# rakhimovv/lvt

Measured on AMD Instinct MI355X. Metric: video-clips/sec/node (VQVAE+DSFVT train step, BAIR 64x64x16), higher is better.
Workload: dtype f32

## Files before the change

### lvt_amd/csrc/gemm_engine.hip

```cpp
#include "lvt_common.h"
#include "epilogue_fast.h"
#include <string.h>
#include <stdlib.h>
#include <stdint.h>
#include <type_traits>

typedef float f32x16 __attribute__((ext_vector_type(16)));

#define BK 32
#define NTHREADS 256

enum { A_KPLAIN = 0, A_MPLAIN = 1, A_CONV_K = 2, A_CONVT_K = 3, A_CONV_M = 4, A_ONEHOT_M = 5, A_PATCH = 6, A_PATCHT = 7 };
enum { B_KPLAIN = 0, B_NPLAIN = 1, B_CONVT_W = 2 };

struct KParams {
    int M, N, K;
    const float *A; long long lda; int a_kb; long long a_skb;
    const float *B; long long ldb; int b_kb; long long b_skb;
    float *C; long long ldc; long long c_plane;
    int batch_inner;
    long long sA_o, sA_i, sB_o, sB_i, sC_o, sC_i;
    float alpha; int flags;
    const float *bias; const float *res; long long ldr; const float *mask; long long ldm;
    int splits; int k_per_split; float *partial; long long partial_stride;
    int vec_epi;
    float *colsum_partial;
    const float *a_amax, *b_amax;
    const float *a_amax2, *b_amax2;
    float *c_amax;
    lvt_conv_geom g;
    const char *b_img;
    int Tq, Hq, Wq;
    int jT, jH, jW;
    const long long *oh_idx; long long oh_bstride, oh_pstride; int oh_P, oh_V; int oh_off[32];
};

__device__ __forceinline__ float4 ldg4(const float *p) { return *reinterpret_cast<const float4 *>(p); }

__device__ __forceinline__ unsigned cvt_pk_bf16(float lo, float hi) {
    unsigned r;
    asm("v_cvt_pk_bf16_f32 %0, %1, %2" : "=v"(r) : "v"(lo), "v"(hi));
    return r;
}
__device__ __forceinline__ float bf_lo(unsigned p) { return __uint_as_float(p << 16); }
__device__ __forceinline__ float bf_hi(unsigned p) { return __uint_as_float(p & 0xffff0000u); }
__device__ __forceinline__ void split3(const float4 v, uint2 &p1, uint2 &p2, uint2 &p3) {
    p1.x = cvt_pk_bf16(v.x, v.y); p1.y = cvt_pk_bf16(v.z, v.w);
    const float r0 = v.x - bf_lo(p1.x), r1 = v.y - bf_hi(p1.x), r2 = v.z - bf_lo(p1.y), r3 = v.w - bf_hi(p1.y);
    p2.x = cvt_pk_bf16(r0, r1); p2.y = cvt_pk_bf16(r2, r3);
    const float s0 = r0 - bf_lo(p2.x), s1 = r1 - bf_hi(p2.x), s2 = r2 - bf_lo(p2.y), s3 = r3 - bf_hi(p2.y);
    p3.x = cvt_pk_bf16(s0, s1); p3.y = cvt_pk_bf16(s2, s3);
}
#define HLD 40
template <int ROWS> __device__ __forceinline__ int hrow(int m) {
    if (ROWS >= 128) {
        const int r = (m & ~127) + ((m & 3) << 5) + ((m & 127) >> 2);
        return r * HLD + (r >> 5) * 32;
    }
    return m * HLD;
}
template <int ROWS> struct HPlane { static constexpr int SIZE = ROWS * HLD + (ROWS >= 128 ? ROWS : 0); };
template <int ROWS> __device__ __forceinline__ void store_split_k(unsigned short *lds, int row, int k4, const float4 v) {
    uint2 p1, p2, p3;
    split3(v, p1, p2, p3);
    unsigned short *d = lds + hrow<ROWS>(row) + k4;
    *reinterpret_cast<uint2 *>(d) = p1;
    *reinterpret_cast<uint2 *>(d + HPlane<ROWS>::SIZE) = p2;
    *reinterpret_cast<uint2 *>(d + 2 * HPlane<ROWS>::SIZE) = p3;
}
template <int ROWS> __device__ __forceinline__ void store_split_m(unsigned short *lds, int row4, int k, const float4 v) {
    uint2 p[3];
    split3(v, p[0], p[1], p[2]);
#pragma unroll
    for (int q = 0; q < 3; ++q) {
        unsigned short *d = lds + q * HPlane<ROWS>::SIZE + k;
        d[hrow<ROWS>(row4)] = (unsigned short)(p[q].x & 0xffffu); d[hrow<ROWS>(row4 + 1)] = (unsigned short)(p[q].x >> 16);
        d[hrow<ROWS>(row4 + 2)] = (unsigned short)(p[q].y & 0xffffu); d[hrow<ROWS>(row4 + 3)] = (unsigned short)(p[q].y >> 16);
    }
}
template <int ROWS> __device__ __forceinline__ void store_split_block(unsigned short *lds, int row4, int k4, const float4 *v) {
    store_split_k<ROWS>(lds, row4 + 0, k4, make_float4(v[0].x, v[1].x, v[2].x, v[3].x));
    store_split_k<ROWS>(lds, row4 + 1, k4, make_float4(v[0].y, v[1].y, v[2].y, v[3].y));
    store_split_k<ROWS>(lds, row4 + 2, k4, make_float4(v[0].z, v[1].z, v[2].z, v[3].z));
    store_split_k<ROWS>(lds, row4 + 3, k4, make_float4(v[0].w, v[1].w, v[2].w, v[3].w));
}
__device__ __forceinline__ float4 zero4() { return make_float4(0.f, 0.f, 0.f, 0.f); }

typedef float f32x2 __attribute__((ext_vector_type(2)));
typedef _Float16 f16x2v __attribute__((ext_vector_type(2)));
__device__ __forceinline__ float f16_mix_lo(unsigned h, float k, float c) {
    float r;
    asm("v_fma_mix_f32 %0, %1, %2, %3 op_sel:[0,0,0] op_sel_hi:[1,0,0]" : "=v"(r) : "v"(h), "v"(k), "v"(c));
    return r;
}
__device__ __forceinline__ float f16_mix_hi(unsigned h, float k, float c) {
    float r;
    asm("v_fma_mix_f32 %0, %1, %2, %3 op_sel:[1,0,0] op_sel_hi:[1,0,0]" : "=v"(r) : "v"(h), "v"(k), "v"(c));
    return r;
}
template <int LOSCALE>
__device__ __forceinline__ void f16_split_pair(float a, float b, float s, unsigned &ph, unsigned &pl) {
    const f32x2 v = {a, b};
    ph = __builtin_bit_cast(unsigned, __builtin_convertvector(v * s, f16x2v));
    const f32x2 t2 = v * (s * (float)LOSCALE);
    const f32x2 r = {f16_mix_lo(ph, -(float)LOSCALE, t2.x), f16_mix_hi(ph, -(float)LOSCALE, t2.y)};
    pl = __builtin_bit_cast(unsigned, __builtin_convertvector(r, f16x2v));
}
__device__ __forceinline__ void split2(const float4 v, const float s, uint2 &ph, uint2 &pl) {
    f16_split_pair<2048>(v.x, v.y, s, ph.x, pl.x);
    f16_split_pair<2048>(v.z, v.w, s, ph.y, pl.y);
}
__device__ __forceinline__ unsigned f16_pair_mix(float a, float b, float s) {
    unsigned r;
    asm("v_fma_mixlo_f16 %0, %1, %2, 0\n\tv_fma_mixhi_f16 %0, %3, %2, 0" : "=&v"(r) : "v"(a), "v"(s), "v"(b));
    return r;
}
__device__ __forceinline__ void split2_lean(const float4 v, const float s, uint2 &ph, uint2 &pl) {
    ph.x = f16_pair_mix(v.x, v.y, s); ph.y = f16_pair_mix(v.z, v.w, s);
    pl.x = f16_pair_mix(f16_mix_lo(ph.x, -1.f, v.x * s), f16_mix_hi(ph.x, -1.f, v.y * s), 2048.f);
    pl.y = f16_pair_mix(f16_mix_lo(ph.y, -1.f, v.z * s), f16_mix_hi(ph.y, -1.f, v.w * s), 2048.f);
}
__device__ __forceinline__ float lvt_f16_scale(const float *amax, int &unscale, const float *amax2 = nullptr) {
    if (!amax) return 1.f;
    unsigned bits = __float_as_uint(*amax);
    if (amax2) bits = max(bits, __float_as_uint(*amax2));
    const int eb = (int)((bits >> 23) & 0xffu);
    int se = 268 - eb;
    se = se < 2 ? 2 : (se > 252 ? 252 : se);
    unscale -= se - 127;
    return __uint_as_float((unsigned)se << 23);
}
template <int ROWS, int LEAN = 0> __device__ __forceinline__ void store_split2_k(unsigned short *lds, int row, int k4, const float4 v, float s) {
    uint2 ph, pl;
    if (LEAN) split2_lean(v, s, ph, pl);
    else split2(v, s, ph, pl);
    unsigned short *d = lds + hrow<ROWS>(row) + k4;
    *reinterpret_cast<uint2 *>(d) = ph;
    *reinterpret_cast<uint2 *>(d + HPlane<ROWS>::SIZE) = pl;
}
template <int ROWS, int LEAN = 0> __device__ __forceinline__ void store_split2_m(unsigned short *lds, int row4, int k, const float4 v, float s) {
    uint2 p[2];
    if (LEAN) split2_lean(v, s, p[0], p[1]);
    else split2(v, s, p[0], p[1]);
#pragma unroll
    for (int q = 0; q < 2; ++q) {
        unsigned short *d = lds + q * HPlane<ROWS>::SIZE + k;
        d[hrow<ROWS>(row4)] = (unsigned short)(p[q].x & 0xffffu); d[hrow<ROWS>(row4 + 1)] = (unsigned short)(p[q].x >> 16);
        d[hrow<ROWS>(row4 + 2)] = (unsigned short)(p[q].y & 0xffffu); d[hrow<ROWS>(row4 + 3)] = (unsigned short)(p[q].y >> 16);
    }
}
template <int ROWS, int LEAN = 0> __device__ __forceinline__ void store_split2_block(unsigned short *lds, int row4, int k4, const float4 *v, float s) {
    store_split2_k<ROWS, LEAN>(lds, row4 + 0, k4, make_float4(v[0].x, v[1].x, v[2].x, v[3].x), s);
    store_split2_k<ROWS, LEAN>(lds, row4 + 1, k4, make_float4(v[0].y, v[1].y, v[2].y, v[3].y), s);
    store_split2_k<ROWS, LEAN>(lds, row4 + 2, k4, make_float4(v[0].z, v[1].z, v[2].z, v[3].z), s);
    store_split2_k<ROWS, LEAN>(lds, row4 + 3, k4, make_float4(v[0].w, v[1].w, v[2].w, v[3].w), s);
}

struct Cursor4 {
    int c, w, h, t;
    __device__ __forceinline__ void seek(int k, int nC, int nW, int nH) {
        int q = k / nC; c = k - q * nC;
        w = q % nW; q /= nW;
        h = q % nH; t = q / nH;
    }
    __device__ __forceinline__ void advance(int step, int nC, int nW, int nH) {
        c += step;
        while (c >= nC) {
            c -= nC;
            if (++w == nW) { w = 0; if (++h == nH) { h = 0; ++t; } }
        }
    }
};

template <int MODE, int BM, int MATH> struct ALoader;

#define QPR (BK / 4)
#define RPP (NTHREADS / QPR)
#define KPAD 1
template <int MODE, int BM> struct AKLoaderBase {
    static constexpr int ITERS = BM / RPP;
    static constexpr int LD = BM + KPAD;
    float4 v[ITERS];
    int r0, kq;
    __device__ __forceinline__ void store(float *lds) const {
#pragma unroll
        for (int i = 0; i < ITERS; ++i) {
            const int row = r0 + RPP * i;
            lds[(kq * 4 + 0) * LD + row] = v[i].x;
            lds[(kq * 4 + 1) * LD + row] = v[i].y;
            lds[(kq * 4 + 2) * LD + row] = v[i].z;
            lds[(kq * 4 + 3) * LD + row] = v[i].w;
        }
    }
    __device__ __forceinline__ void store_split(unsigned short *lds) const {
#pragma unroll
        for (int i = 0; i < ITERS; ++i) store_split_k<BM>(lds, r0 + RPP * i, kq * 4, v[i]);
    }
    __device__ __forceinline__ void store_split2(unsigned short *lds, float s) const {
#pragma unroll
        for (int i = 0; i < ITERS; ++i) store_split2_k<BM>(lds, r0 + RPP * i, kq * 4, v[i], s);
    }
};

template <int BM, int MATH> struct ALoader<A_KPLAIN, BM, MATH> : AKLoaderBase<A_KPLAIN, BM> {
    using Base = AKLoaderBase<A_KPLAIN, BM>;
    const float *rowp[Base::ITERS];
    bool rowok[Base::ITERS];
    int kb, kcur, kin; long long skb, kbase;
    __device__ __forceinline__ void init(const KParams &p, int tid, int m0, const float *A, int) {
        this->r0 = tid / QPR; this->kq = tid % QPR;
        kb = p.a_kb; skb = p.a_skb;
#pragma unroll
        for (int i = 0; i < Base::ITERS; ++i) {
            const int m = m0 + this->r0 + RPP * i;
            rowok[i] = m < p.M;
            rowp[i] = A + (long long)m * p.lda;
        }
    }
    __device__ __forceinline__ void seek(int k0) {
        kcur = k0 + this->kq * 4;
        const int blk = kcur / kb;
        kin = kcur - blk * kb; kbase = (long long)blk * skb;
    }
    __device__ __forceinline__ void fetch(int kend) {
        const bool kok = kcur < kend;
        const long long koff = kbase + kin;
#pragma unroll
        for (int i = 0; i < Base::ITERS; ++i)
            this->v[i] = (kok && rowok[i]) ? ldg4(rowp[i] + koff) : zero4();
        kcur += BK; kin += BK;
        while (kin >= kb) { kin -= kb; kbase += skb; }
    }
};

template <int BM, int MATH> struct ALoader<A_CONV_K, BM, MATH> : AKLoaderBase<A_CONV_K, BM> {
    using Base = AKLoaderBase<A_CONV_K, BM>;
    const float *rowp[Base::ITERS];
    int ti0[Base::ITERS], hi0[Base::ITERS], wi0[Base::ITERS];
    int Ci, Kw, Kh, Ti, Hi, Wi, kcur;
    Cursor4 cur;
    __device__ __forceinline__ void init(const KParams &p, int tid, int m0, const float *A, int) {
        this->r0 = tid / QPR; this->kq = tid % QPR;
        const lvt_conv_geom &g = p.g;
        Ci = g.Ci; Kw = g.Kw; Kh = g.Kh; Ti = g.Ti; Hi = g.Hi; Wi = g.Wi;
#pragma unroll
        for (int i = 0; i < Base::ITERS; ++i) {
            int m = m0 + this->r0 + RPP * i;
            if (m < p.M) {
                const int wo = m % g.Wo; m /= g.Wo;
                const int ho = m % g.Ho; m /= g.Ho;
                const int to = m % g.To; const int n = m / g.To;
                ti0[i] = to * g.st - g.pt; hi0[i] = ho * g.sh - g.ph; wi0[i] = wo * g.sw - g.pw;
                rowp[i] = A + ((((long long)n * Ti + ti0[i]) * Hi + hi0[i]) * Wi + wi0[i]) * Ci;
            } else {
                ti0[i] = -(1 << 28); hi0[i] = 0; wi0[i] = 0; rowp[i] = A;
            }
        }
    }
    __device__ __forceinline__ void seek(int k0) {
        kcur = k0 + this->kq * 4;
        cur.seek(kcur, Ci, Kw, Kh);
    }
    __device__ __forceinline__ void fetch(int kend) {
        const bool kok = kcur < kend;
        const int tapoff = ((cur.t * Hi + cur.h) * Wi + cur.w) * Ci + cur.c;
#pragma unroll
        for (int i = 0; i < Base::ITERS; ++i) {
            const bool ok = kok && (unsigned)(ti0[i] + cur.t) < (unsigned)Ti && (unsigned)(hi0[i] + cur.h) < (unsigned)Hi &&
                            (unsigned)(wi0[i] + cur.w) < (unsigned)Wi;
            this->v[i] = ok ? ldg4(rowp[i] + tapoff) : zero4();
        }
        kcur += BK;
        cur.advance(BK, Ci, Kw, Kh);
    }
};

template <int BM, int MATH> struct ALoader<A_CONVT_K, BM, MATH> : AKLoaderBase<A_CONVT_K, BM> {
    using Base = AKLoaderBase<A_CONVT_K, BM>;
    const float *rowp[Base::ITERS];
    int ot0[Base::ITERS], oh0[Base::ITERS], ow0[Base::ITERS];
    int Co, jH, jW, To, Ho, Wo, kcur;
    Cursor4 cur;
    __device__ __forceinline__ void init(const KParams &p, int tid, int m0, const float *A, int cls) {
        this->r0 = tid / QPR; this->kq = tid % QPR;
        const lvt_conv_geom &g = p.g;
        Co = g.Co; jH = p.jH; jW = p.jW; To = g.To; Ho = g.Ho; Wo = g.Wo;
        const int fw = cls % g.sw, fh = (cls / g.sw) % g.sh, ft = cls / (g.sw * g.sh);
        const int rt = ((ft - g.pt) % g.st + g.st) % g.st, ct = (rt + g.pt - ft) / g.st;
        const int rh = ((fh - g.ph) % g.sh + g.sh) % g.sh, ch = (rh + g.ph - fh) / g.sh;
        const int rw = ((fw - g.pw) % g.sw + g.sw) % g.sw, cw = (rw + g.pw - fw) / g.sw;
#pragma unroll
// ... 870 lines not shown
    const float *bcol = p.B + n0 + bnq * 4;
    float4 bv[4];
    auto b_fetch = [&](int step) {
        const int cc = step / NTAPS, tap = step - cc * NTAPS;
        const int wrow = MODE == 2 ? ((cc & 3) * NTAPS + tap) * Ci + (cc >> 2) * 32 : (phase * NTAPS + tap) * Ci + cc * 32;
        const float *src = bcol + (long long)(wrow + bkk0 * 4) * p.ldb;
#pragma unroll
        for (int i = 0; i < 4; ++i) bv[i] = ldg4(src + (long long)i * p.ldb);
    };

    f32x16 acc[TM][TN];
    f32x16 acx[MATH == 2 ? TM : 1][MATH == 2 ? TN : 1];
#pragma unroll
    for (int i = 0; i < TM; ++i)
#pragma unroll
        for (int j = 0; j < TN; ++j)
#pragma unroll
            for (int r = 0; r < 16; ++r) {
                acc[i][j][r] = 0.f;
                if (MATH == 2) acx[i][j][r] = 0.f;
            }
    auto b_store = [&](unsigned short *dst) {
        if (MATH == 2) store_split2_block<BN>(dst, bnq * 4, bkk0 * 4, bv, sb);
        else store_split_block<BN>(dst, bnq * 4, bkk0 * 4, bv);
    };
    const int wave_s = __builtin_amdgcn_readfirstlane(wave);
    constexpr int B_UNITS = PT_BIMG_BYTES / 16;
    static_assert(PT_BIMG_BYTES == NP * PSB * 2 || !BIMG, "image = the LDS buffer");
    const char *bimg0 = BIMG ? p.b_img + (long long)(n0 / BN) * PT_BIMG_BYTES + tid * 16 : nullptr;
    auto b_dma = [&](int step, unsigned short *dst) {
        const int cc = step / NTAPS, tap = step - cc * NTAPS;
        const int wrow = MODE == 2 ? ((cc & 3) * NTAPS + tap) * Ci + (cc >> 2) * 32 : (phase * NTAPS + tap) * Ci + cc * 32;
        const char *src = bimg0 + (long long)(wrow >> 5) * ntn * PT_BIMG_BYTES;
        char *d = reinterpret_cast<char *>(dst) + wave_s * 1024;
        __builtin_amdgcn_global_load_lds((pt_gl_void *)src, (pt_lds_void *)d, 16, 0, 0);
        __builtin_amdgcn_global_load_lds((pt_gl_void *)(src + 8192), (pt_lds_void *)(d + 8192), 16, 0, 0);
        if (tid + 1024 < B_UNITS) __builtin_amdgcn_global_load_lds((pt_gl_void *)(src + 16384), (pt_lds_void *)(d + 16384), 16, 0, 0);
    };
    const int b_nprobe = wave_s * 64 + 1024 < B_UNITS ? 3 : 2;
    const unsigned b_probe = (unsigned)((lane % b_nprobe) * 8192 + wave_s * 1024 + (lane & 31) * 16);
    auto b_landed = [&](const unsigned short *dst) {
        asm volatile("s_waitcnt vmcnt(0)" ::: "memory");
        const int v = *reinterpret_cast<const volatile int *>(reinterpret_cast<const char *>(dst) + b_probe);
        (void)v;
        asm volatile("s_waitcnt lgkmcnt(0)" ::: "memory");
    };

    int arow[TM];
    {
        const int q = l31 >> 2, e = l31 & 3;
        const int yy = __popc(q) & 1, x = 4 * (q >> 1) + e;
#pragma unroll
        for (int i = 0; i < TM; ++i) arow[i] = ((2 * (2 * wm + i) + yy) * PT_PW + x) * HLD + 8 * half;
    }
    int brow[TN];
#pragma unroll
    for (int j = 0; j < TN; ++j) brow[j] = hrow<BN>(wn * (TN * 32) + j * 32 + l31) + 8 * half;

    const int nchunks = (Ci / 32) * (MODE == 2 ? 4 : 1), nsteps = nchunks * NTAPS;
    patch_fetch(0);
    if (BIMG) b_dma(0, Bh0);
    else if (bact) b_fetch(0);
    patch_store(Ah);
    if (BIMG) b_landed(Bh0);
    else if (bact) b_store(Bh0);
    __syncthreads();

    for (int step = 0; step < nsteps; ++step) {
        const int cc = step / NTAPS, tap = step - cc * NTAPS;
        const bool has_next = step + 1 < nsteps;
        const bool new_chunk = has_next && tap == NTAPS - 1;
        if (BIMG) { if (has_next) b_dma(step + 1, Bh0 + ((step + 1) & 1) * (NP * PSB)); }
        else if (has_next && bact) b_fetch(step + 1);
        if (DBLA ? (cc + 1 < nchunks && tap == NTAPS - 2) : new_chunk) patch_fetch(cc + 1);
        const unsigned short *Bh = Bh0 + (step & 1) * (NP * PSB);
        const unsigned short *Acur = Ah + (DBLA ? (cc & 1) * A_IMG : 0);
        const unsigned short *Ap = MODE == 0 ? Acur + ((tap / 3) * PT_PW + (tap % 3)) * HLD
                                             : Acur + (((phase >> 1) + (tap >> 1)) * PT_PW + (phase & 1) + (tap & 1)) * HLD;
        if constexpr (MATH == 2) {
#pragma unroll
            for (int ks = 0; ks < BK; ks += 16) {
                f16x8 a[2][TM], b[2][TN];
#pragma unroll
                for (int q = 0; q < 2; ++q) {
#pragma unroll
                    for (int i = 0; i < TM; ++i) a[q][i] = *reinterpret_cast<const f16x8 *>(Ap + arow[i] + q * PT_PLANE + ks);
#pragma unroll
                    for (int j = 0; j < TN; ++j) b[q][j] = *reinterpret_cast<const f16x8 *>(Bh + brow[j] + q * PSB + ks);
                }
#pragma unroll
                for (int i = 0; i < TM; ++i)
#pragma unroll
                    for (int j = 0; j < TN; ++j)
                        acx[i][j] = __builtin_amdgcn_mfma_f32_32x32x16_f16(a[0][i], b[1][j], acx[i][j], 0, 0, 0);
#pragma unroll
                for (int i = 0; i < TM; ++i)
#pragma unroll
                    for (int j = 0; j < TN; ++j)
                        acc[i][j] = __builtin_amdgcn_mfma_f32_32x32x16_f16(a[0][i], b[0][j], acc[i][j], 0, 0, 0);
#pragma unroll
                for (int i = 0; i < TM; ++i)
#pragma unroll
                    for (int j = 0; j < TN; ++j)
                        acx[i][j] = __builtin_amdgcn_mfma_f32_32x32x16_f16(a[1][i], b[0][j], acx[i][j], 0, 0, 0);
            }
            if (DBLA && new_chunk) patch_store(Ah + ((cc + 1) & 1) * A_IMG);
        } else {
#pragma unroll
            for (int ks = 0; ks < BK; ks += 16) {
                bf16x8 a[3][TM], b[3][TN];
#pragma unroll
                for (int q = 0; q < 3; ++q) {
#pragma unroll
                    for (int i = 0; i < TM; ++i) a[q][i] = *reinterpret_cast<const bf16x8 *>(Ap + arow[i] + q * PT_PLANE + ks);
#pragma unroll
                    for (int j = 0; j < TN; ++j) b[q][j] = *reinterpret_cast<const bf16x8 *>(Bh + brow[j] + q * PSB + ks);
                }
                constexpr int TA[6] = {1, 0, 2, 0, 1, 0}, TB[6] = {1, 2, 0, 1, 0, 0};
#pragma unroll
                for (int t = 0; t < 6; ++t)
#pragma unroll
                    for (int i = 0; i < TM; ++i)
#pragma unroll
                        for (int j = 0; j < TN; ++j)
                            acc[i][j] = __builtin_amdgcn_mfma_f32_32x32x16_bf16(a[TA[t]][i], b[TB[t]][j], acc[i][j], 0, 0, 0);
            }
        }
        if (!BIMG && has_next && bact) b_store(Bh0 + ((step + 1) & 1) * (NP * PSB));
        if (!DBLA && new_chunk) {
            __syncthreads();
            patch_store(Ah);
        }
        if (BIMG && has_next) b_landed(Bh0 + ((step + 1) & 1) * (NP * PSB));
        __syncthreads();
    }
    if constexpr (MATH == 2) lvt_f16x2_finish<TM, TN>(acc, acx, unscale);
    if (p.vec_epi && p.splits <= 1 && !(p.flags & (LVT_EPI_PLANES | LVT_EPI_ACCUM | LVT_EPI_TANH | LVT_EPI_SIGMOID))) {
        const unsigned seen = lvt_amax_peek(p.c_amax);
        LvtEpi e;
        e.M = p.M; e.N = p.N; e.C = p.C; e.ldc = p.ldc; e.coff = 0; e.alpha = p.alpha; e.flags = p.flags;
        e.bias = p.bias; e.res = p.res; e.ldr = p.ldr; e.mask = p.mask; e.ldm = p.ldm;
        float *wave_tile = lds + wave * (32 * TN * 32);
        float am_w;
        if (MODE != 1) am_w = lvt_epi_fast_dispatch<TM, TN, PatchRows>(e, acc, wave_tile, m0 + wm * (TM * 32), n0 + wn * (TN * 32), lane, PatchRows());
        else am_w = lvt_epi_fast_dispatch<TM, TN, PatchTRows>(e, acc, wave_tile, m0 + wm * (TM * 32), n0 + wn * (TN * 32), lane, PatchTRows{phase});
        if (p.c_amax) lvt_block_amax_commit_seen(am_w, p.c_amax, lds + TURN_FLOATS, seen);
        return;
    }
    if (MODE != 1) lvt_epilogue_vec<A_PATCH, BM, BN, WM, WN>(p, acc, lds, m0, n0, wm, wn, lane, 0, 0, 0, 0);
    else lvt_epilogue_vec<A_PATCHT, BM, BN, WM, WN>(p, acc, lds, m0, n0, wm, wn, lane, phase, 0, 0, 0);
}

#define WIDE_THREADS 512
template <int TA, int TB>
__global__ __launch_bounds__(WIDE_THREADS, 2) void lvt_gemm_wide_kernel(const KParams p) {
    constexpr int BM = 256, BN = 128, WM = 4, WN = 2, TM = 2, TN = 2;
    constexpr int AMODE = TA ? A_MPLAIN : A_KPLAIN;
    constexpr int PSA = HPlane<BM>::SIZE, PSB = HPlane<BN>::SIZE;
    constexpr int STAGE = 2 * (PSA + PSB);
    constexpr int STAGE_FLOATS = (2 * STAGE) / 2 + 8;
    constexpr int TURN_FLOATS = WM * WN * 32 * (TN * 32);
    constexpr int LDS_FLOATS = STAGE_FLOATS > TURN_FLOATS ? STAGE_FLOATS : TURN_FLOATS;
    __shared__ __attribute__((aligned(16))) float lds[LDS_FLOATS];
    unsigned short *S0 = reinterpret_cast<unsigned short *>(lds);

    const int tid = threadIdx.x, lane = tid & 63, wave = tid >> 6;
    const int wm = wave / WN, wn = wave % WN;
    const int l31 = lane & 31, half = lane >> 5;
    const TileCtx tc = lvt_tile_ctx<AMODE, BM, BN>(p);
    const int m0 = tc.m0, n0 = tc.n0, kbeg = tc.kbeg, kend = tc.kend;

    int unscale = 0;
    const float sa = lvt_f16_scale(p.a_amax, unscale, p.a_amax2), sb = lvt_f16_scale(p.b_amax, unscale, p.b_amax2);

    float4 av[4], bv[TB ? 4 : 2];
    const int r0 = tid >> 3, kq = tid & 7;
    const int kk0 = TA ? tid >> 6 : 0, mq = tid & 63;
    const int bkk0 = (tid >> 5) & 7, bnq = tid & 31;
    const bool bact = !TB || tid < 256;
    const char *Ak = reinterpret_cast<const char *>(tc.A), *Bk = reinterpret_cast<const char *>(tc.B);
    unsigned aoff[4], boff_g[TB ? 4 : 2];
    int a_kin = 0, b_kin = 0;
    if (!TA) {
#pragma unroll
        for (int i = 0; i < 4; ++i) aoff[i] = (unsigned)(((long long)min(m0 + r0 + 64 * i, p.M - 1) * p.lda + kq * 4) * 4);
        const int blk = kbeg / p.a_kb;
        a_kin = kbeg - blk * p.a_kb;
        Ak += ((long long)blk * p.a_skb + a_kin) * 4;
    } else {
        const int m = m0 + mq * 4;
#pragma unroll
        for (int i = 0; i < 4; ++i) aoff[i] = (unsigned)(((long long)(kk0 * 4 + i) * p.lda + (m < p.M ? m : 0)) * 4);
        Ak += (long long)kbeg * p.lda * 4;
    }
    if (!TB) {
#pragma unroll
        for (int i = 0; i < 2; ++i) boff_g[i] = (unsigned)(((long long)min(n0 + r0 + 64 * i, p.N - 1) * p.ldb + kq * 4) * 4);
        const int blk = kbeg / p.b_kb;
        b_kin = kbeg - blk * p.b_kb;
        Bk += ((long long)blk * p.b_skb + b_kin) * 4;
    } else {
        const int n = n0 + bnq * 4;
#pragma unroll
        for (int i = 0; i < 4; ++i) boff_g[i] = (unsigned)(((long long)(bkk0 * 4 + i) * p.ldb + (n < p.N ? n : 0)) * 4);
        Bk += (long long)kbeg * p.ldb * 4;
    }
    const bool sum_on = TA && p.colsum_partial != nullptr && n0 == 0;
    float4 colacc = zero4();
    auto fetch = [&]() {
#pragma unroll
        for (int i = 0; i < 4; ++i) av[i] = *reinterpret_cast<const float4 *>(Ak + aoff[i]);
        if (!TA) {
            a_kin += BK;
            const bool wrap = a_kin >= p.a_kb;
            Ak += wrap ? ((long long)p.a_skb - p.a_kb + BK) * 4 : (long long)BK * 4;
            a_kin = wrap ? 0 : a_kin;
        } else {
            Ak += (long long)BK * p.lda * 4;
            if (sum_on) {
#pragma unroll
                for (int i = 0; i < 4; ++i) { colacc.x += av[i].x; colacc.y += av[i].y; colacc.z += av[i].z; colacc.w += av[i].w; }
            }
        }
        if (!TB) {
#pragma unroll
            for (int i = 0; i < 2; ++i) bv[i] = *reinterpret_cast<const float4 *>(Bk + boff_g[i]);
            b_kin += BK;
            const bool wrap = b_kin >= p.b_kb;
            Bk += wrap ? ((long long)p.b_skb - p.b_kb + BK) * 4 : (long long)BK * 4;
            b_kin = wrap ? 0 : b_kin;
        } else {
            if (bact) {
#pragma unroll
                for (int i = 0; i < 4; ++i) bv[i] = *reinterpret_cast<const float4 *>(Bk + boff_g[i]);
            }
            Bk += (long long)BK * p.ldb * 4;
        }
    };
    auto store = [&](unsigned short *buf) {
        unsigned short *Ah = buf, *Bh = buf + 2 * PSA;
        if (!TA) {
#pragma unroll
            for (int i = 0; i < 4; ++i) store_split2_k<BM>(Ah, r0 + 64 * i, kq * 4, av[i], sa);
        } else {
            store_split2_block<BM>(Ah, mq * 4, kk0 * 4, av, sa);
        }
        if (!TB) {
#pragma unroll
            for (int i = 0; i < 2; ++i) store_split2_k<BN>(Bh, r0 + 64 * i, kq * 4, bv[i], sb);
        } else if (bact) {
            store_split2_block<BN>(Bh, bnq * 4, bkk0 * 4, bv, sb);
        }
    };

    f32x16 acc[TM][TN], acx[TM][TN];
#pragma unroll
    for (int i = 0; i < TM; ++i)
#pragma unroll
        for (int j = 0; j < TN; ++j)
#pragma unroll
            for (int r = 0; r < 16; ++r) { acc[i][j][r] = 0.f; acx[i][j][r] = 0.f; }

    int fa[TM], fb[TN];
#pragma unroll
    for (int i = 0; i < TM; ++i) fa[i] = hrow<BM>(wm * (TM * 32) + i * 32 + l31) + 8 * half;
#pragma unroll
    for (int j = 0; j < TN; ++j) fb[j] = 2 * PSA + hrow<BN>(wn * (TN * 32) + j * 32 + l31) + 8 * half;

    auto tile = [&](const unsigned short *cur, unsigned short *nxt, auto do_store, auto do_fetch) {
#pragma unroll
        for (int ks = 0; ks < BK; ks += 16) {
            f16x8 a[2][TM], b[2][TN];
#pragma unroll
            for (int q = 0; q < 2; ++q) {
#pragma unroll
                for (int i = 0; i < TM; ++i) a[q][i] = *reinterpret_cast<const f16x8 *>(cur + fa[i] + q * PSA + ks);
#pragma unroll
                for (int j = 0; j < TN; ++j) b[q][j] = *reinterpret_cast<const f16x8 *>(cur + fb[j] + q * PSB + ks);
            }
#pragma unroll
            for (int i = 0; i < TM; ++i)
#pragma unroll
                for (int j = 0; j < TN; ++j)
                    acx[i][j] = __builtin_amdgcn_mfma_f32_32x32x16_f16(a[0][i], b[1][j], acx[i][j], 0, 0, 0);
#pragma unroll
            for (int i = 0; i < TM; ++i)
#pragma unroll
                for (int j = 0; j < TN; ++j)
                    acc[i][j] = __builtin_amdgcn_mfma_f32_32x32x16_f16(a[0][i], b[0][j], acc[i][j], 0, 0, 0);
#pragma unroll
            for (int i = 0; i < TM; ++i)
#pragma unroll
                for (int j = 0; j < TN; ++j)
                    acx[i][j] = __builtin_amdgcn_mfma_f32_32x32x16_f16(a[1][i], b[0][j], acx[i][j], 0, 0, 0);
            if (ks == 0) {
                if constexpr (decltype(do_store)::value) store(nxt);
                if constexpr (decltype(do_fetch)::value) fetch();
            }
        }
    };
    typedef std::integral_constant<bool, true> yes_t;
    typedef std::integral_constant<bool, false> no_t;

    const int ntiles = kbeg < kend ? (kend - kbeg) / BK : 0;
    if (ntiles > 0) {
        fetch();
        store(S0);
        if (ntiles > 1) fetch();
    }
    __syncthreads();
    int kt = 0;
    for (; kt + 2 < ntiles; ++kt) {
        tile(S0 + (kt & 1) * STAGE, S0 + ((kt + 1) & 1) * STAGE, yes_t(), yes_t());
        __syncthreads();
    }
    if (kt + 1 < ntiles) {
        tile(S0 + (kt & 1) * STAGE, S0 + ((kt + 1) & 1) * STAGE, yes_t(), no_t());
        __syncthreads();
        ++kt;
    }
    if (kt < ntiles) tile(S0 + (kt & 1) * STAGE, nullptr, no_t(), no_t());
    __syncthreads();
    lvt_f16x2_finish<TM, TN>(acc, acx, unscale);

    if (TA && sum_on) {
        float *scratch = lds;
        *reinterpret_cast<float4 *>(&scratch[(kk0 * 64 + mq) * 4]) = colacc;
        __syncthreads();
        if (tid < BM) {
            float s_ = 0.f;
            for (int r = 0; r < 8; ++r) s_ += scratch[(r * 64 + tid / 4) * 4 + (tid & 3)];
            if (m0 + tid < p.M) p.colsum_partial[((long long)tc.split * gridDim.y + tc.z) * p.M + m0 + tid] = s_;
        }
        __syncthreads();
    }
    if (p.vec_epi && !(p.flags & (LVT_EPI_PLANES | LVT_EPI_ACCUM | LVT_EPI_TANH | LVT_EPI_SIGMOID))) {
        LvtEpi e;
        e.M = p.M; e.N = p.N;
        float *wave_tile = lds + wave * (32 * TN * 32);
        if (p.splits > 1) {
            e.C = p.partial; e.ldc = p.N; e.coff = tc.split * p.partial_stride + (long long)tc.z * p.M * p.N; e.alpha = 1.f; e.flags = 0;
            e.bias = nullptr; e.res = nullptr; e.ldr = 0; e.mask = nullptr; e.ldm = 0;
            (void)lvt_epi_fast_wave<0, TM, TN>(e, acc, wave_tile, m0 + wm * (TM * 32), n0 + wn * (TN * 32), lane);
            return;
        }
        const unsigned seen = lvt_amax_peek(p.c_amax);
        e.C = p.C; e.ldc = p.ldc; e.coff = tc.coff; e.alpha = p.alpha; e.flags = p.flags;
        e.bias = p.bias; e.res = p.res; e.ldr = p.ldr; e.mask = p.mask; e.ldm = p.ldm;
        const float am_w = lvt_epi_fast_dispatch<TM, TN>(e, acc, wave_tile, m0 + wm * (TM * 32), n0 + wn * (TN * 32), lane);
        if (p.c_amax) lvt_block_amax_commit_seen(am_w, p.c_amax, lds + TURN_FLOATS, seen);
        return;
    }
    if (p.vec_epi) lvt_epilogue_vec<AMODE, BM, BN, WM, WN>(p, acc, lds, m0, n0, wm, wn, lane, 0, tc.coff, tc.z, tc.split);
    else lvt_epilogue<AMODE, BM, BN, WM, WN>(p, acc, m0, n0, wm, wn, l31, half, 0, tc.coff, tc.z, tc.split);
}

__global__ void lvt_reduce_splits_kernel(const float *__restrict__ partial, long long n4, long long stride,
                                         int splits, float *__restrict__ out, int accumulate) {
    long long i = (long long)blockIdx.x * blockDim.x + threadIdx.x;
    const long long step = (long long)gridDim.x * blockDim.x;
    for (; i < n4; i += step) {
        float4 s0 = ldg4(partial + i * 4), s1 = zero4(), s2 = zero4(), s3 = zero4();
        int k = 1;
        for (; k + 3 < splits; k += 4) {
            const float4 t0 = ldg4(partial + k * stride + i * 4), t1 = ldg4(partial + (k + 1) * stride + i * 4);
            const float4 t2 = ldg4(partial + (k + 2) * stride + i * 4), t3 = ldg4(partial + (k + 3) * stride + i * 4);
            s0.x += t0.x; s0.y += t0.y; s0.z += t0.z; s0.w += t0.w;
            s1.x += t1.x; s1.y += t1.y; s1.z += t1.z; s1.w += t1.w;
            s2.x += t2.x; s2.y += t2.y; s2.z += t2.z; s2.w += t2.w;
            s3.x += t3.x; s3.y += t3.y; s3.z += t3.z; s3.w += t3.w;
        }
        for (; k < splits; ++k) {
            const float4 t = ldg4(partial + k * stride + i * 4);
            s0.x += t.x; s0.y += t.y; s0.z += t.z; s0.w += t.w;
        }
        float4 s;
        s.x = (s0.x + s1.x) + (s2.x + s3.x); s.y = (s0.y + s1.y) + (s2.y + s3.y);
        s.z = (s0.z + s1.z) + (s2.z + s3.z); s.w = (s0.w + s1.w) + (s2.w + s3.w);
        float4 *o = reinterpret_cast<float4 *>(out + i * 4);
        if (accumulate) { const float4 c = *o; s.x += c.x; s.y += c.y; s.z += c.z; s.w += c.w; }
        *o = s;
    }
}

__global__ void lvt_pack_weight_kernel(const float *__restrict__ w, float *__restrict__ wp, int taps, int Ci,
                                       int Co, int Ci_real, int Co_real) {
    const long long total = (long long)taps * Ci * Co;
    for (long long i = (long long)blockIdx.x * blockDim.x + threadIdx.x; i < total;
         i += (long long)gridDim.x * blockDim.x) {
        const int co = i % Co; long long t = i / Co;
        const int ci = t % Ci; const int tap = t / Ci;
        float v = 0.f;
        if (co < Co_real && ci < Ci_real) v = w[((long long)co * Ci_real + ci) * taps + tap];
        wp[i] = v;
    }
}
__global__ void lvt_pack_weight_t_kernel(const float *__restrict__ w, float *__restrict__ wt, int taps, int Ci,
                                         int Co, int Ci_real, int Co_real) {
    const long long total = (long long)taps * Co * Ci;
    for (long long i = (long long)blockIdx.x * blockDim.x + threadIdx.x; i < total;
         i += (long long)gridDim.x * blockDim.x) {
        const int ci = i % Ci; long long t = i / Ci;
        const int co = t % Co; const int tr = t / Co;
        float v = 0.f;
        if (co < Co_real && ci < Ci_real) v = w[((long long)co * Ci_real + ci) * taps + (taps - 1 - tr)];
        wt[i] = v;
    }
}
__global__ void lvt_pack_weight_phases_kernel(const float *__restrict__ w, float *__restrict__ wph, int Ci, int Co,
                                              int Ci_real, int Co_real) {
    const long long total = 16LL * Co * Ci;
    for (long long i = (long long)blockIdx.x * blockDim.x + threadIdx.x; i < total; i += (long long)gridDim.x * blockDim.x) {
        const int ci = i % Ci; long long t = i / Ci;
        const int co = t % Co; const int pt = t / Co;
        const int ph = pt >> 2, tap = pt & 3;
        const int ky = 3 - (ph >> 1) - 2 * (tap >> 1), kx = 3 - (ph & 1) - 2 * (tap & 1);
        float v = 0.f;
        if (co < Co_real && ci < Ci_real) v = w[(((long long)co * Ci_real + ci) * 4 + ky) * 4 + kx];
        wph[i] = v;
    }
}
__global__ void lvt_pack_weight_parity_kernel(const float *__restrict__ w, float *__restrict__ wq, int Ci, int Co,
                                              int Ci_real, int Co_real) {
    const long long total = 16LL * Ci * Co;
    for (long long i = (long long)blockIdx.x * blockDim.x + threadIdx.x; i < total; i += (long long)gridDim.x * blockDim.x) {
        const int co = i % Co; long long t = i / Co;
        const int ci = t % Ci; const int ct = t / Ci;
        const int cls = ct >> 2, tap = ct & 3;
        const int ky = 2 * (tap >> 1) + (cls >> 1), kx = 2 * (tap & 1) + (cls & 1);
        float v = 0.f;
        if (co < Co_real && ci < Ci_real) v = w[(((long long)co * Ci_real + ci) * 4 + ky) * 4 + kx];
// ... 796 lines not shown
```

Measured before the change: 1362.

## Use ds_read_tr16 transposed LDS layout for transposed operands in wide GEMM

For transposed A/B inputs (M- or N-contiguous), the wide GEMM kernel now stores the split fp16 hi/lo planes in a K-major padded LDS image. It then reads MFMA fragments with the hardware transpose-read instruction ds_read_tr16_b64, instead of scattering per-element transposing stores. This removes the 4x4 register transpose and the narrow LDS writes on the store side. It also lets all 512 threads load B in the TB case, rather than only half of them. The cost is a larger padded LDS footprint and a dependence on the fragment offset mapping being exactly right.

```diff
diff --git a/lvt_amd/csrc/gemm_engine.hip b/lvt_amd/csrc/gemm_engine.hip
--- a/lvt_amd/csrc/gemm_engine.hip
+++ b/lvt_amd/csrc/gemm_engine.hip
@@ -1,5 +1,6 @@
 #include "lvt_common.h"
 #include "epilogue_fast.h"
+#include "wide_image.h"
 #include <string.h>
 #include <stdlib.h>
 #include <stdint.h>
@@ -137,6 +138,12 @@
     unsigned short *d = lds + hrow<ROWS>(row) + k4;
     *reinterpret_cast<uint2 *>(d) = ph;
     *reinterpret_cast<uint2 *>(d + HPlane<ROWS>::SIZE) = pl;
+}
+template <int PLANE> __device__ __forceinline__ void store_split2_tr(unsigned short *d, const float4 v, float s) {
+    uint2 ph, pl;
+    split2(v, s, ph, pl);
+    *reinterpret_cast<uint2 *>(d) = ph;
+    *reinterpret_cast<uint2 *>(d + PLANE) = pl;
 }
 template <int ROWS, int LEAN = 0> __device__ __forceinline__ void store_split2_m(unsigned short *lds, int row4, int k, const float4 v, float s) {
     uint2 p[2];
@@ -1313,11 +1320,20 @@
 }
 
 #define WIDE_THREADS 512
+typedef short s16x4 __attribute__((ext_vector_type(4)));
+template <int PITCH> __device__ __forceinline__ f16x8 wide_tr_frag(const unsigned short *p) {
+    typedef __attribute__((address_space(3))) s16x4 lds_v4;
+    union { struct { s16x4 a, b; } s; f16x8 v; } u;
+    u.s.a = __builtin_amdgcn_ds_read_tr16_b64_v4i16((lds_v4 *)(p));
+    u.s.b = __builtin_amdgcn_ds_read_tr16_b64_v4i16((lds_v4 *)(p + 4 * PITCH));
+    return u.v;
+}
 template <int TA, int TB>
 __global__ __launch_bounds__(WIDE_THREADS, 2) void lvt_gemm_wide_kernel(const KParams p) {
     constexpr int BM = 256, BN = 128, WM = 4, WN = 2, TM = 2, TN = 2;
     constexpr int AMODE = TA ? A_MPLAIN : A_KPLAIN;
-    constexpr int PSA = HPlane<BM>::SIZE, PSB = HPlane<BN>::SIZE;
+    constexpr int PA = wide_tr_pitch(BM), PB = wide_tr_pitch(BN);
+    constexpr int PSA = TA ? wide_tr_plane(BM) : HPlane<BM>::SIZE, PSB = TB ? wide_tr_plane(BN) : HPlane<BN>::SIZE;
     constexpr int STAGE = 2 * (PSA + PSB);
     constexpr int STAGE_FLOATS = (2 * STAGE) / 2 + 8;
     constexpr int TURN_FLOATS = WM * WN * 32 * (TN * 32);
@@ -1334,13 +1350,12 @@
     int unscale = 0;
     const float sa = lvt_f16_scale(p.a_amax, unscale, p.a_amax2), sb = lvt_f16_scale(p.b_amax, unscale, p.b_amax2);
 
-    float4 av[4], bv[TB ? 4 : 2];
+    float4 av[4], bv[2];
     const int r0 = tid >> 3, kq = tid & 7;
     const int kk0 = TA ? tid >> 6 : 0, mq = tid & 63;
-    const int bkk0 = (tid >> 5) & 7, bnq = tid & 31;
-    const bool bact = !TB || tid < 256;
+    const int bk0 = tid >> 5, bnq = tid & 31;
     const char *Ak = reinterpret_cast<const char *>(tc.A), *Bk = reinterpret_cast<const char *>(tc.B);
-    unsigned aoff[4], boff_g[TB ? 4 : 2];
+    unsigned aoff[4], boff_g[2];
     int a_kin = 0, b_kin = 0;
     if (!TA) {
 #pragma unroll
@@ -1363,7 +1378,7 @@
     } else {
         const int n = n0 + bnq * 4;
 #pragma unroll
-        for (int i = 0; i < 4; ++i) boff_g[i] = (unsigned)(((long long)(bkk0 * 4 + i) * p.ldb + (n < p.N ? n : 0)) * 4);
+        for (int i = 0; i < 2; ++i) boff_g[i] = (unsigned)(((long long)(bk0 + 16 * i) * p.ldb + (n < p.N ? n : 0)) * 4);
         Bk += (long long)kbeg * p.ldb * 4;
     }
     const bool sum_on = TA && p.colsum_partial != nullptr && n0 == 0;
@@ -1383,34 +1398,28 @@
                 for (int i = 0; i < 4; ++i) { colacc.x += av[i].x; colacc.y += av[i].y; colacc.z += av[i].z; colacc.w += av[i].w; }
             }
         }
+#pragma unroll
+        for (int i = 0; i < 2; ++i) bv[i] = *reinterpret_cast<const float4 *>(Bk + boff_g[i]);
         if (!TB) {
-#pragma unroll
-            for (int i = 0; i < 2; ++i) bv[i] = *reinterpret_cast<const float4 *>(Bk + boff_g[i]);
             b_kin += BK;
             const bool wrap = b_kin >= p.b_kb;
             Bk += wrap ? ((long long)p.b_skb - p.b_kb + BK) * 4 : (long long)BK * 4;
             b_kin = wrap ? 0 : b_kin;
         } else {
-            if (bact) {
-#pragma unroll
-                for (int i = 0; i < 4; ++i) bv[i] = *reinterpret_cast<const float4 *>(Bk + boff_g[i]);
-            }
             Bk += (long long)BK * p.ldb * 4;
         }
     };
     auto store = [&](unsigned short *buf) {
         unsigned short *Ah = buf, *Bh = buf + 2 * PSA;
-        if (!TA) {
-#pragma unroll
-            for (int i = 0; i < 4; ++i) store_split2_k<BM>(Ah, r0 + 64 * i, kq * 4, av[i], sa);
-        } else {
-            store_split2_block<BM>(Ah, mq * 4, kk0 * 4, av, sa);
-        }
-        if (!TB) {
-#pragma unroll
-            for (int i = 0; i < 2; ++i) store_split2_k<BN>(Bh, r0 + 64 * i, kq * 4, bv[i], sb);
-        } else if (bact) {
-            store_split2_block<BN>(Bh, bnq * 4, bkk0 * 4, bv, sb);
+#pragma unroll
+        for (int i = 0; i < 4; ++i) {
+            if (!TA) store_split2_k<BM>(Ah, r0 + 64 * i, kq * 4, av[i], sa);
+            else store_split2_tr<PSA>(Ah + wide_tr_store_off(BM, kk0 * 4 + i, mq * 4), av[i], sa);
+        }
+#pragma unroll
+        for (int i = 0; i < 2; ++i) {
+            if (!TB) store_split2_k<BN>(Bh, r0 + 64 * i, kq * 4, bv[i], sb);
+            else store_split2_tr<PSB>(Bh + wide_tr_store_off(BN, bk0 + 16 * i, bnq * 4), bv[i], sb);
         }
     };
 
@@ -1424,9 +1433,11 @@
 
     int fa[TM], fb[TN];
 #pragma unroll
-    for (int i = 0; i < TM; ++i) fa[i] = hrow<BM>(wm * (TM * 32) + i * 32 + l31) + 8 * half;
-#pragma unroll
-    for (int j = 0; j < TN; ++j) fb[j] = 2 * PSA + hrow<BN>(wn * (TN * 32) + j * 32 + l31) + 8 * half;
+    for (int i = 0; i < TM; ++i)
+        fa[i] = TA ? wide_tr_frag_off(BM, lane, wm * (TM * 32) + i * 32) : hrow<BM>(wm * (TM * 32) + i * 32 + l31) + 8 * half;
+#pragma unroll
+    for (int j = 0; j < TN; ++j)
+        fb[j] = 2 * PSA + (TB ? wide_tr_frag_off(BN, lane, wn * (TN * 32) + j * 32) : hrow<BN>(wn * (TN * 32) + j * 32 + l31) + 8 * half);
 
     auto tile = [&](const unsigned short *cur, unsigned short *nxt, auto do_store, auto do_fetch) {
 #pragma unroll
@@ -1435,9 +1446,15 @@
 #pragma unroll
             for (int q = 0; q < 2; ++q) {
 #pragma unroll
-                for (int i = 0; i < TM; ++i) a[q][i] = *reinterpret_cast<const f16x8 *>(cur + fa[i] + q * PSA + ks);
-#pragma unroll
-                for (int j = 0; j < TN; ++j) b[q][j] = *reinterpret_cast<const f16x8 *>(cur + fb[j] + q * PSB + ks);
+                for (int i = 0; i < TM; ++i) {
+                    if (TA) a[q][i] = wide_tr_frag<PA>(cur + fa[i] + q * PSA + ks * PA);
+                    else a[q][i] = *reinterpret_cast<const f16x8 *>(cur + fa[i] + q * PSA + ks);
+                }
+#pragma unroll
+                for (int j = 0; j < TN; ++j) {
+                    if (TB) b[q][j] = wide_tr_frag<PB>(cur + fb[j] + q * PSB + ks * PB);
+                    else b[q][j] = *reinterpret_cast<const f16x8 *>(cur + fb[j] + q * PSB + ks);
+                }
             }
 #pragma unroll
             for (int i = 0; i < TM; ++i)
diff --git a/lvt_amd/csrc/wide_image.h b/lvt_amd/csrc/wide_image.h
--- /dev/null
+++ b/lvt_amd/csrc/wide_image.h
@@ -0,0 +1,14 @@
+#pragma once
+#if defined(__HIPCC__)
+#define LVT_WIDE_HD __host__ __device__
+#else
+#define LVT_WIDE_HD
+#endif
+
+#define WIDE_TR_ROWS 32
+LVT_WIDE_HD constexpr int wide_tr_pitch(int cols) { return cols + 32; }
+LVT_WIDE_HD constexpr int wide_tr_plane(int cols) { return WIDE_TR_ROWS * wide_tr_pitch(cols); }
+LVT_WIDE_HD constexpr int wide_tr_store_off(int cols, int k, int col4) { return k * wide_tr_pitch(cols) + col4; }
+LVT_WIDE_HD constexpr int wide_tr_frag_off(int cols, int lane, int col0) {
+    return (8 * (lane >> 5) + ((lane & 15) >> 2)) * wide_tr_pitch(cols) + col0 + 16 * ((lane >> 4) & 1) + 4 * (lane & 3);
+}
```

Result: no change. 1367 (median of 6 runs) (+0.4%).
